# liron88/HM-16.2

Measured on AMD Instinct MI355X. Metric: CTUs/sec (enc) at 4K main10; bit-exact CU partition vs HM, higher is better.
Workload: dtype int32+f64

## Files before the change

### hm-16.2_amd/csrc/hm355_core.h

```cpp
#pragma once
#include <stddef.h>
#include "hm355_types.h"

#ifdef HM355_HOSTSIM
#include <string.h>
#include <math.h>
#include <stdlib.h>
#define HM_DEV static
#define HM_FINL static inline
#define HM_FINL_M inline
#define HM_LAMBDA_INL
#define HM_NOINLINE __attribute__((noinline))
#define HM_CONST static const
#define HM_ASSUME_LDS(p) ((void)0)
#define HM_ASSUME_GLB(p) ((void)0)
#define HM_NT 1
static inline int hm_lane() { return 0; }
#define HM_SYNC() ((void)0)
static inline uint32_t hm_wave_sum(uint32_t v) { return v; }
static inline int hm_wave_sum_i(int v) { return v; }
static inline int hm_wave_max_i(int v) { return v; }
#define HM_UNI(x) (x)
#define HM_UCALL(x) (x)
#define hm_uni_ptr(p) (p)
// ... 45 lines not shown
}
__device__ __forceinline__ uint32_t hm_wave_sum(uint32_t v) { return (uint32_t)hm_wave_sum_i((int)v); }
__device__ __forceinline__ int hm_wave_max_i(int v)
{
  int t;
  t = hm_dpp<0x111>(v, v); v = t > v ? t : v; t = hm_dpp<0x112>(v, v); v = t > v ? t : v;
  t = hm_dpp<0x114>(v, v); v = t > v ? t : v; t = hm_dpp<0x118>(v, v); v = t > v ? t : v;
  const int a = __builtin_amdgcn_readlane(v, 15), b = __builtin_amdgcn_readlane(v, 31), c = __builtin_amdgcn_readlane(v, 47), d = __builtin_amdgcn_readlane(v, 63);
  const int ab = a > b ? a : b, cd = c > d ? c : d;
  return ab > cd ? ab : cd;
}
#define HM_LDS_ADD(p, v) atomicAdd((p), (v))
#define HM_UNI(x) __builtin_amdgcn_readfirstlane((int)(x))
template <class T> __device__ __forceinline__ T *hm_uni_ptr(T *p)
{
  const unsigned long long v = (unsigned long long)p;
  const unsigned lo = (unsigned)__builtin_amdgcn_readfirstlane((int)(unsigned)v), hi = (unsigned)__builtin_amdgcn_readfirstlane((int)(unsigned)(v >> 32));
  return (T *)(((unsigned long long)hi << 32) | lo);
}
template <class T> __device__ __forceinline__ T hm_uni_struct(T v)
{
  static_assert(sizeof(T) % 4 == 0, "dword-sized aggregates only");
  int w[sizeof(T) / 4];
  __builtin_memcpy(w, &v, sizeof(T));
#pragma unroll
  for (unsigned i = 0; i < sizeof(T) / 4; i++) w[i] = __builtin_amdgcn_readfirstlane(w[i]);
  __builtin_memcpy(&v, w, sizeof(T));
  return v;
}
#define HM_ENTRY(e) do { (e) = hm_uni_ptr(e); HM_ASSUME_LDS(e); } while (0)
#define HM_UCALL(x) ((uint32_t)__builtin_amdgcn_readfirstlane((int)(x)))
#define HM_PAR_FOR(i, n) for (int i = hm_lane(); i < (n); i += HM_NT)
#define HM_PAR_FOR_XY(x, y, w, n) \
  for (int i_ = hm_lane(), sy_ = HM_NT / (w), sx_ = HM_NT - sy_ * (w), y = i_ / (w), x = i_ - y * (w); i_ < (n); \
       i_ += HM_NT, x += sx_, y += sy_, (x >= (w) ? (x -= (w), y++) : 0))
#define HM_WAVE_FOR(k) for (int k = hm_lane(), k##_once = 1; k##_once; k##_once = 0)
#define HM_LV(T, name) T name
#define HM_LVARG(T, name) const T name
#define HM_LVK(name, k) name
#define HM_LV_GET(name, i) __builtin_amdgcn_readlane((int)(name), (int)(i))
#define HM_LV_GETD(name, i) hm_readlane_d((name), (int)(i))
#define HM_LV_SET(name, i, v) ((name) = (hm_lane() == (int)(i)) ? (v) : (name))
#define HM_LV_SETD(name, i, v) ((name) = (hm_lane() == (int)(i)) ? (v) : (name))
#define HM_LV_GATHER(name, idx) __builtin_amdgcn_ds_bpermute((int)(idx) << 2, (int)(name))
#define HM_BALLOT(m, k, cond) ((m) = __ballot(cond))
#define HM_ORDERED_ADD16(acc, name) do { _Pragma("unroll") for (int k_ = 15; k_ >= 0; k_--) (acc) += hm_readlane_d((name), k_); } while (0)
#define HM_ORDERED_CHAIN16(acc, a, b, pre) do { _Pragma("unroll") for (int k_ = 15; k_ >= 0; k_--) { \
    (pre) = (hm_lane() == k_) ? (acc) : (pre); (acc) -= hm_readlane_d((a), k_); (acc) += hm_readlane_d((b), k_); } } while (0)
__device__ __forceinline__ double hm_readlane_d(double v, int i)
{ return __hiloint2double(__builtin_amdgcn_readlane(__double2hiint(v), i), __builtin_amdgcn_readlane(__double2loint(v), i)); }
#endif

#if defined(HM355_PROFILE) && !defined(HM355_HOSTSIM)
#define HM_PROF_N 45
#define HM_PROF_BEGIN(e, id) const unsigned long long prof_t0_##id = __builtin_readcyclecounter()
#define HM_PROF_END(e, id) do { (e)->prof[id] += __builtin_readcyclecounter() - prof_t0_##id; (e)->profCnt[id] += 1; } while (0)
#else
#define HM_PROF_BEGIN(e, id) ((void)0)
#define HM_PROF_END(e, id) ((void)0)
#endif
enum { PR_RDOQ = 0, PR_BITS, PR_ADI, PR_PRED, PR_FWD, PR_INV, PR_SATD35, PR_TUBLK, PR_SAVE, PR_CHROMA, PR_LUMA, PR_ENCCU, PR_TOTAL,
       PR_S4L = 32, PR_S4C, PR_D0, PR_D1, PR_D2, PR_D3, PR_NXN, PR_S8L, PR_S4LEAF, PR_S4CLEAF, PR_S8C, PR_S16L = 44,
       PR_ME_INT = 16, PR_ME_FRAC, PR_AMVP, PR_MRG_EST, PR_MC, PR_IRQ, PR_IRES, PR_MRG2N, PR_INTERCU, PR_INTRA_IN_P, PR_IQ_FULL, PR_IQ_FWD, PR_IQ_RDOQ, PR_IQ_BITS, PR_IQ_INV, PR_IQ_ENC };

#define HM_MAX_DOUBLE 1.7e+308
#define PLANAR_IDX 0
#define DC_IDX 1
#define HOR_IDX 10
#define VER_IDX 26
#define DM_CHROMA_IDX 36
#define SIZE_2Nx2N 0
#define SIZE_NxN 3
#define SIZE_NONE 8
#define MODE_INTRA 1
#define MODE_NONE 2
#define SCAN_DIAG 0
#define SCAN_HOR 1
#define SCAN_VER 2

HM_CONST uint8_t HM_NEXT_LPS[128] __attribute__((aligned(4))) = {
  1, 0, 0, 1, 2, 3, 4, 5, 4, 5, 8, 9, 8, 9, 10, 11, 12, 13, 14, 15, 16, 17, 18, 19, 18, 19, 22, 23, 22, 23, 24, 25,
  26, 27, 26, 27, 30, 31, 30, 31, 32, 33, 32, 33, 36, 37, 36, 37, 38, 39, 38, 39, 42, 43, 42, 43, 44, 45, 44, 45, 46, 47, 48, 49,
  48, 49, 50, 51, 52, 53, 52, 53, 54, 55, 54, 55, 56, 57, 58, 59, 58, 59, 60, 61, 60, 61, 60, 61, 62, 63, 64, 65, 64, 65, 66, 67,
  66, 67, 66, 67, 68, 69, 68, 69, 70, 71, 70, 71, 70, 71, 72, 73, 72, 73, 72, 73, 74, 75, 74, 75, 74, 75, 76, 77, 76, 77, 126, 127 };
HM_CONST int32_t HM_ENTROPY_BITS[128] = {
  0x07b23, 0x085f9, 0x074a0, 0x08cbc, 0x06ee4, 0x09354, 0x067f4, 0x09c1b, 0x060b0, 0x0a62a, 0x05a9c, 0x0af5b, 0x0548d, 0x0b955, 0x04f56, 0x0c2a9,
  0x04a87, 0x0cbf7, 0x045d6, 0x0d5c3, 0x04144, 0x0e01b, 0x03d88, 0x0e937, 0x039e0, 0x0f2cd, 0x03663, 0x0fc9e, 0x03347, 0x10600, 0x03050, 0x10f95,
  0x02d4d, 0x11a02, 0x02ad3, 0x12333, 0x0286e, 0x12cad, 0x02604, 0x136df, 0x02425, 0x13f48, 0x021f4, 0x149c4, 0x0203e, 0x1527b, 0x01e4d, 0x15d00,
  0x01c99, 0x166de, 0x01b18, 0x17017, 0x019a5, 0x17988, 0x01841, 0x18327, 0x016df, 0x18d50, 0x015d9, 0x19547, 0x0147c, 0x1a083, 0x0138e, 0x1a8a3,
  0x01251, 0x1b418, 0x01166, 0x1bd27, 0x01068, 0x1c77b, 0x00f7f, 0x1d18e, 0x00eda, 0x1d91a, 0x00e19, 0x1e254, 0x00d4f, 0x1ec9a, 0x00c90, 0x1f6e0,
  0x00c01, 0x1fef8, 0x00b5f, 0x208b1, 0x00ab6, 0x21362, 0x00a15, 0x21e46, 0x00988, 0x2285d, 0x00934, 0x22ea8, 0x008a8, 0x239b2, 0x0081d, 0x24577,
  0x007c9, 0x24ce6, 0x00763, 0x25663, 0x00710, 0x25e8f, 0x006a0, 0x26a26, 0x00672, 0x26f23, 0x005e8, 0x27ef8, 0x005ba, 0x284b5, 0x0055e, 0x29057,
  0x0050c, 0x29bab, 0x004c1, 0x2a674, 0x004a7, 0x2aa5e, 0x0046f, 0x2b32f, 0x0041f, 0x2c0ad, 0x003e7, 0x2ca8d, 0x003ba, 0x2d323, 0x0010c, 0x3bfbb };
HM_CONST uint8_t HM_CTX_INIT_I[HM_NUM_CTX] = {
   139, 141, 157,
   184, 154, 154, 154,
   184,
   63, 139,
   153, 138, 138,
   111, 141, 154, 154, 154,   94, 138, 182, 154, 154,
   91, 171, 134, 141,
   111, 111, 125, 110, 110, 94, 124, 108, 124, 107, 125, 141, 179, 153, 125, 107, 125, 141, 179, 153, 125, 107, 125, 141, 179, 153, 125, 141,
   140, 139, 182, 182, 152, 136, 152, 136, 153, 136, 139, 111, 136, 139, 111, 111,
   110, 110, 124, 125, 140, 153, 125, 127, 140, 109, 111, 143, 127, 111, 79,  108, 123, 63, 154, 154, 154, 154, 154, 154, 154, 154, 154, 154, 154, 154,
   110, 110, 124, 125, 140, 153, 125, 127, 140, 109, 111, 143, 127, 111, 79,  108, 123, 63, 154, 154, 154, 154, 154, 154, 154, 154, 154, 154, 154, 154,
   140, 92, 137, 138, 140, 152, 138, 139, 153, 74, 149, 92, 139, 107, 122, 152,  140, 179, 166, 182, 140, 227, 122, 197,
   138, 153, 136, 167, 152, 152,
   139, 139,
   154, 154, 154,  154, 154,  154,  154, 154, 154, 154, 154,  154, 154,
   154, 154,  154,  154,  154, 154, 154
};
HM_CONST uint8_t HM_CTX_INIT_P[HM_NUM_CTX] = {
   107, 139, 126,
   154, 139, 154, 154,
   154,
// ... 1580 lines not shown
      const int c = hm_clip3(imin, imax, coef[i]);
      int v;
      if (rightShift > 0) v = (c * scale + (1 << (rightShift - 1))) >> rightShift;
      else v = (int)((unsigned)(c * scale) << (-rightShift));
      e->bufA[y * HM_TSTRIDE + x] = hm_clip3(-32768, 32767, v);
    }
    HM_SYNC();
    if (!tskip) inv_transform(e, n, comp == 0 && n == 4, bitDepth);
    const int off = tshift == 0 ? 0 : (1 << (tshift - 1));
    HM_PAR_FOR(i, n * n) {
      const int y = i >> l2, x = i & (n - 1);
      const int v = e->bufA[y * HM_TSTRIDE + x];
      resi[y * st + x] = (Pel)(tskip ? ((v + off) >> tshift) : v);
    }
  } else {
    HM_PAR_FOR(i, n * n) { const int y = i >> l2, x = i & (n - 1); coef[i] = 0; resi[y * st + x] = 0; }
  }
  HM_SYNC();
  HM_PROF_END(e, PR_INV);
  const int maxv = (1 << bitDepth) - 1, shiftSse = (bitDepth - 8) << 1;
  uint32_t sse = 0;
  HM_PAR_FOR(i, n * n) {
    const int y = i >> l2, x = i & (n - 1);
    const int r = hm_clip3(0, maxv, pred[y * st + x] + resi[y * st + x]);
    pred[y * st + x] = (Pel)r; recQt[y * st + x] = (Pel)r; recPic[y * ps + x] = (Pel)r;
    const int d = org[y * ps + x] - r; sse += (uint32_t)((d * d) >> shiftSse);
  }
  uint32_t d = hm_wave_sum(sse);
  HM_SYNC();
  if (comp) d = (uint32_t)(e->fb.chromaWeight * (double)d);
  return d;
}

HM_DEV inline void store_intra_result_qt(Shared *e, const TU *t, int comp)
{
  const int st = HM_PLANE_STRIDE(comp), po = HM_PLANE_OFF(comp), layer = 5 - t->log2;
  const int bx = comp ? t->cx : t->x, by = comp ? t->cy : t->y;
  const TCoeff *coef = e->ws->qtCoef[layer] + po + (comp ? t->cOff : (t->cuZ + t->relZ) * 16);
  const Pel *rq = e->ws->qtRec[layer] + po + by * st + bx;
  HM_PAR_FOR(i, 16) { e->ws->tsCoef[comp][i] = coef[i]; e->ws->tsRec[comp][i] = rq[(i >> 2) * st + (i & 3)]; }
  HM_SYNC();
}
HM_DEV inline void load_intra_result_qt(Shared *e, const TU *t, int comp)
{
  const int st = HM_PLANE_STRIDE(comp), po = HM_PLANE_OFF(comp), layer = 5 - t->log2, ps = e->stride[comp];
  const int bx = comp ? t->cx : t->x, by = comp ? t->cy : t->y;
  TCoeff *coef = e->ws->qtCoef[layer] + po + (comp ? t->cOff : (t->cuZ + t->relZ) * 16);
  Pel *rq = e->ws->qtRec[layer] + po + by * st + bx;
  Pel *recPic = e->fb.rec[comp] + (e->ctuY * st + by) * ps + e->ctuX * st + bx;
  HM_PAR_FOR(i, 16) { coef[i] = e->ws->tsCoef[comp][i]; const Pel v = e->ws->tsRec[comp][i]; rq[(i >> 2) * st + (i & 3)] = v; recPic[(i >> 2) * ps + (i & 3)] = v; }
  HM_SYNC();
}

HM_DEV HM_NOINLINE void simt4_luma_leaf(Shared *e, TU tv);
template <int L2> HM_DEV HM_NOINLINE void simt_luma_winner_as_single_tu(Shared *e, TU tv);
HM_DEV HM_NOINLINE void recur_intra_coding_qt(Shared *e, TU rootv, int checkFirst)
{
  HM_ENTRY(e); checkFirst = HM_UNI(checkFirst); rootv = hm_uni_struct(rootv);
  CtuMeta *m = (&e->meta);
  RqtFrame *fr = e->rqt; int sp = 0;
  uint32_t *retDist = e->rqtRetDist, *retBits = e->rqtRetBits; double *retCost = e->rqtRetCost;
  fr[0].t = rootv; fr[0].phase = 0; retDist[0] = 0; retBits[0] = 0; retCost[0] = 0.0;
  while (sp >= 0) {
    RqtFrame *f = &fr[sp]; const TU *t = &f->t;
    const int z = t->cuZ + t->relZ, fullDepth = t->cuDepth + t->trDepth, log2 = t->log2;
    if (f->phase == 0) {
      const int nxn = m->part[t->cuZ] == SIZE_NxN;
      f->checkFull = log2 <= 5;
      f->checkSplit = log2 > tr_min_size_in_cu(6 - t->cuDepth, nxn);
      if (checkFirst && f->checkFull) f->checkSplit = 0;
      f->singleCost = HM_MAX_DOUBLE; f->singleDist = 0; f->singleCbf = 0; f->bestModeId = 0; f->singleBits = 0;
      const int checkTS = (log2 == 2) && (m->part[z] == SIZE_NxN);
      if (f->checkFull) {
        if (checkTS) {
          cabac_copy(&e->ws->slot[HM_SLOT(fullDepth, CI_QT_TRAFO_ROOT)], &e->cur);
          for (int modeId = 0; modeId < 2; modeId++) {
            double costTmp;
            par_set8(m->ts[0] + z, modeId, t->parts);
            const uint32_t distTmp = HM_UCALL(intra_coding_tu_block(e, *t, 0, modeId == 0 ? 1 : 2));
            const uint32_t cbfTmp = (m->cbf[0][z] >> t->trDepth) & 1;
            if (modeId == 1 && cbfTmp == 0) costTmp = HM_MAX_DOUBLE;
            else { const uint32_t bits = HM_UCALL(intra_bits_qt(e, *t, 1, 0)); costTmp = calc_rd_cost(e, bits, distTmp); }
            if (costTmp < f->singleCost) {
              f->singleCost = costTmp; f->singleDist = distTmp; f->singleCbf = cbfTmp; f->bestModeId = (int8_t)modeId;
              if (modeId == 0) { store_intra_result_qt(e, t, 0); cabac_copy(&e->ws->slot[HM_SLOT(fullDepth, CI_TEMP_BEST)], &e->cur); }
            }
            if (modeId == 0) cabac_copy(&e->cur, &e->ws->slot[HM_SLOT(fullDepth, CI_QT_TRAFO_ROOT)]);
          }
          par_set8(m->ts[0] + z, f->bestModeId, t->parts);
          if (f->bestModeId == 0) {
            load_intra_result_qt(e, t, 0);
            par_set8(m->cbf[0] + z, (int)(f->singleCbf << t->trDepth), t->parts);
            cabac_copy(&e->cur, &e->ws->slot[HM_SLOT(fullDepth, CI_TEMP_BEST)]);
          }
        } else if (log2 == 2 && e->P->fewWaves) {
          par_set8(m->ts[0] + z, 0, t->parts);
          HM_PROF_BEGIN(e, PR_S4LEAF);
          simt4_luma_leaf(e, *t);
          HM_PROF_END(e, PR_S4LEAF);
          f->singleDist = e->outDistY; f->singleBits = e->outBits;
          f->singleCost = calc_rd_cost(e, e->outBits, f->singleDist);
        } else if (sp == 0 && e->s8Reuse == 1) {
          e->s8Reuse = 0;
          cabac_copy(&e->ws->slot[HM_SLOT(fullDepth, CI_QT_TRAFO_ROOT)], &e->cur);
          par_set8(m->ts[0] + z, 0, t->parts);
          par_set8(m->tr + z, t->trDepth, t->parts);
          if (log2 == 3) simt_luma_winner_as_single_tu<3>(e, *t); else simt_luma_winner_as_single_tu<4>(e, *t);
          f->singleDist = e->outDistY; f->singleCbf = e->outDist;
          par_set8(m->cbf[0] + z, (int)(f->singleCbf << t->trDepth), t->parts);
          f->singleCost = calc_rd_cost(e, e->outBits, f->singleDist);
        } else if (sp == 0 && e->s8Reuse == 2) {
          e->s8Reuse = 0;
          cabac_copy(&e->ws->slot[HM_SLOT(fullDepth, CI_QT_TRAFO_ROOT)], &e->cur);
          par_set8(m->ts[0] + z, 0, t->parts);
          par_set8(m->tr + z, t->trDepth, t->parts);
          {
            const int n = 1 << log2, layer = 5 - log2;
            par_copy32(e->ws->qtCoef[layer] + z * 16, e->cc + z * 16, n * n);
            par_copy_blk(e->ws->qtRec[layer] + t->y * 64 + t->x, 64, e->ws->reco + t->y * 64 + t->x, 64, n);
          }
          f->singleCbf = e->ws->tmpCbf[0][0] & 1;
          par_set8(m->cbf[0] + z, (int)(f->singleCbf << t->trDepth), t->parts);
          f->singleDist = e->outDistY; f->singleCost = e->outRdCost;
          cabac_copy(&e->cur, &e->ws->slot[HM_SLOT(fullDepth, CI_QT_TRAFO_TEST)]);
        } else {
          if (f->checkSplit) cabac_copy(&e->ws->slot[HM_SLOT(fullDepth, CI_QT_TRAFO_ROOT)], &e->cur);
          par_set8(m->ts[0] + z, 0, t->parts);
          f->singleDist = HM_UCALL(intra_coding_tu_block(e, *t, 0, 0));
          if (f->checkSplit) f->singleCbf = (m->cbf[0][z] >> t->trDepth) & 1;
          const uint32_t bits = HM_UCALL(intra_bits_qt(e, *t, 1, 0));
          f->singleCost = calc_rd_cost(e, bits, f->singleDist); f->singleBits = bits;
        }
      }
      if (!f->checkSplit) { retDist[sp] += f->singleDist; retBits[sp] += f->singleBits; retCost[sp] += f->singleCost; sp--; continue; }
      if (f->checkFull) { cabac_copy(&e->ws->slot[HM_SLOT(fullDepth, CI_QT_TRAFO_TEST)], &e->cur); cabac_copy(&e->cur, &e->ws->slot[HM_SLOT(fullDepth, CI_QT_TRAFO_ROOT)]); }
      else cabac_copy(&e->ws->slot[HM_SLOT(fullDepth, CI_QT_TRAFO_ROOT)], &e->cur);
      f->splitCost = 0.0; f->splitDist = 0; f->splitCbf = 0; f->child = 0; f->phase = 1;
      retDist[sp + 1] = 0; retBits[sp + 1] = 0; retCost[sp + 1] = 0.0;
    }
    if (f->phase == 1) {
      int splitLost = 0;
      if (f->child > 0) {
        const TU ch = tu_child(t, f->child - 1, 0);
        f->splitCbf |= (m->cbf[0][ch.cuZ + ch.relZ] >> ch.trDepth) & 1;
        const uint32_t lbBits = retBits[sp + 1] > (uint32_t)f->child ? retBits[sp + 1] - (uint32_t)f->child : 0;
        if (f->checkFull) splitLost = !(calc_rd_cost(e, lbBits, retDist[sp + 1]) < f->singleCost);
        else if (sp == 0 && !(calc_rd_cost(e, lbBits, retDist[1]) < e->outCost)) {
          e->outDistY = 0; e->outRdCost = HM_MAX_DOUBLE; return;
        }
      }
      if (!splitLost) {
        if (f->child < 4) {
          fr[sp + 1].t = tu_child(t, f->child, 0); fr[sp + 1].phase = 0; f->child++;
          sp++; continue;
        }
        f->splitDist = retDist[sp + 1];
        if (f->splitCbf) { HM_PAR_FOR(o, t->parts) m->cbf[0][z + o] |= (uint8_t)(1 << t->trDepth); HM_SYNC(); }
        cabac_copy(&e->cur, &e->ws->slot[HM_SLOT(fullDepth, CI_QT_TRAFO_ROOT)]);
        const uint32_t splitBits = HM_UCALL(intra_bits_qt(e, *t, 1, 0));
        f->splitCost = calc_rd_cost(e, splitBits, f->splitDist);
        if (f->splitCost < f->singleCost) { retDist[sp] += f->splitDist; retBits[sp] += splitBits; retCost[sp] += f->splitCost; sp--; continue; }
      }
      cabac_copy(&e->cur, &e->ws->slot[HM_SLOT(fullDepth, CI_QT_TRAFO_TEST)]);
      par_set8(m->tr + z, t->trDepth, t->parts);
      par_set8(m->cbf[0] + z, (int)(f->singleCbf << t->trDepth), t->parts);
      par_set8(m->ts[0] + z, f->bestModeId, t->parts);
      {
        const int n = 1 << log2, layer = 5 - log2, ps = e->stride[0];
        par_copy_blk(e->fb.rec[0] + (e->ctuY * 64 + t->y) * ps + e->ctuX * 64 + t->x, ps, e->ws->qtRec[layer] + t->y * 64 + t->x, 64, n);
      }
      retDist[sp] += f->singleDist; retBits[sp] += f->singleBits; retCost[sp] += f->singleCost; sp--; continue;
    }
  }
  e->outDistY = retDist[0]; e->outRdCost = retCost[0];
}

HM_DEV inline void set_intra_result_qt(Shared *e, const TU *root)
{
  const CtuMeta *m = (&e->meta);
  for (int rel = root->relZ; rel < root->relZ + root->parts;) {
    const int z = root->cuZ + rel, trd = m->tr[z];
    const int log2 = 6 - root->cuDepth - trd, n = 1 << log2, layer = 5 - log2;
    const int parts = root->cuParts >> (2 * trd) > 0 ? root->cuParts >> (2 * trd) : 1;
    const int r = hm_z2r(z), x = (r & 15) * 4, y = (r >> 4) * 4;
    par_copy32(e->cc + z * 16, e->ws->qtCoef[layer] + z * 16, n * n);
    par_copy_blk(e->ws->reco + y * 64 + x, 64, e->ws->qtRec[layer] + y * 64 + x, 64, n);
    rel += parts;
  }
}

#include "hm355_simt.h"
#include "hm355_simt4.h"
#include "hm355_simt8.h"
#include "hm355_simt16.h"

HM_DEV HM_NOINLINE uint32_t est_intra_pred_qt(Shared *e, int cuZ, int cuDepth)
{
  HM_ENTRY(e); cuZ = HM_UNI(cuZ); cuDepth = HM_UNI(cuDepth);
  CtuMeta *m = (&e->meta); WorkSpace *ws = e->ws;
  const int cuParts = 256 >> (2 * cuDepth);
  const int nxn = m->part[cuZ] == SIZE_NxN;
  const int numPU = nxn ? 4 : 1, puParts = cuParts / numPU;
  const int puLog2 = 6 - cuDepth - nxn, n = 1 << puLog2;
  const int bitDepth = e->bitDepth, ps = e->stride[0];
  uint32_t overallDistY = 0;
  const TU root = tu_root(e, cuZ, cuDepth);
  for (int pu = 0; pu < numPU; pu++) {
    const TU t = nxn ? tu_child(&root, pu, 0) : root;
    const int z = cuZ + t.relZ;
    int numModesForFullRD = HM_INTRA_MODE_NUM_FAST[puLog2 - 1];
    int32_t *rdModeList = e->rdModeList;
    {
      const int r = hm_z2r(z);
      init_adi_pattern(e, 0, e->ctuX * 64 + t.x, e->ctuY * 64 + t.y, n, e->ctuX * 16 + (r & 15), e->ctuY * 16 + (r >> 4), n / 4, 1);
      const Pel *org = e->fb.org[0] + (e->ctuY * 64 + t.y) * ps + e->ctuX * 64 + t.x;
      Pel *pred = ws->pred + t.y * 64 + t.x;
      int preds[HM_NUM_MPM];
      const int numMpm = intra_dir_predictor(e, z, preds);
      e->mpmZ = z; e->mpmNum = numMpm; e->mpmPreds[0] = preds[0]; e->mpmPreds[1] = preds[1]; e->mpmPreds[2] = preds[2];
      const uint64_t frac0 = e->ws->slot[HM_SLOT(cuDepth, CI_CURR_BEST)].frac & 32767;
      const uint8_t st0 = e->ws->slot[HM_SLOT(cuDepth, CI_CURR_BEST)].s[C_INTRA_LUMA];
      HM_PROF_BEGIN(e, PR_SATD35);
      if (n <= 16) satd_all_modes_small(e, org, ps, n);
      else {
        for (int mode = 0; mode < 35; mode++) {
          pred_intra(e, 0, mode, n, use_filtered_refs(0, mode, n), pred, 64);
          const uint32_t sad = dist_hads(org, ps, pred, 64, n, bitDepth);
          if (hm_lane() == 0) e->satd[mode] = sad;
        }
        HM_SYNC();
      }
      {
        HM_LV(double, vCost);
        HM_WAVE_FOR(k) {
          double cost = HM_MAX_DOUBLE;
          if (k < 35) {
            int predIdx = -1;
            for (int i = 0; i < 3; i++) if (k == preds[i]) predIdx = i;
            uint64_t fb = frac0 + (uint64_t)HM_LT()->ebits[st0 ^ (predIdx != -1)];
            fb += (uint64_t)32768 * (uint64_t)(predIdx == -1 ? 5 : (predIdx ? 2 : 1));
            const uint32_t modeBits = (uint32_t)(fb >> 15);
            cost = (double)e->satd[k] + (double)modeBits * e->fb.sqrtLambda;
          }
          HM_LVK(vCost, k) = cost;
        }
        HM_WAVE_FOR(k) {
          const double ck = HM_LVK(vCost, k);
          int rank = 0;
          for (int j = 0; j < 35; j++) { const double cj = HM_LV_GETD(vCost, j); rank += (cj < ck || (cj == ck && j < k)) ? 1 : 0; }
          if (k < 35 && rank < numModesForFullRD) rdModeList[rank] = k;
        }
        HM_SYNC();
      }
      HM_PROF_END(e, PR_SATD35);
      for (int j = 0; j < numMpm; j++) {
        int included = 0;
        for (int i = 0; i < numModesForFullRD; i++) included |= (preds[j] == rdModeList[i]);
        if (!included) rdModeList[numModesForFullRD++] = preds[j];
      }
    }
    if (n == 4) {
      cabac_copy(&e->cur, &e->ws->slot[HM_SLOT(cuDepth, CI_CURR_BEST)]);
      { HM_PROF_BEGIN(e, PR_S4L); simt4_luma_pu(e, t, numModesForFullRD); HM_PROF_END(e, PR_S4L); }
      overallDistY += e->outDistY;
      if (pu != numPU - 1)
        par_copy_blk(e->fb.rec[0] + (e->ctuY * 64 + t.y) * ps + e->ctuX * 64 + t.x, ps, ws->reco + t.y * 64 + t.x, 64, n);
      continue;
    }
    int bestPUMode = 0; uint32_t bestPUDistY = 0; double bestPUCost = HM_MAX_DOUBLE;
    int firstPass = 0;
    if (n == 8 || n == 16) {
      cabac_copy(&e->cur, &e->ws->slot[HM_SLOT(cuDepth, CI_CURR_BEST)]);
      if (n == 8) { HM_PROF_BEGIN(e, PR_S8L); bestPUMode = HM_UCALL(simt_luma_first_pass<3>(e, t, numModesForFullRD)); HM_PROF_END(e, PR_S8L); }
      else { HM_PROF_BEGIN(e, PR_S16L); bestPUMode = HM_UCALL(simt_luma_first_pass<4>(e, t, numModesForFullRD)); HM_PROF_END(e, PR_S16L); }
      firstPass = numModesForFullRD;
      e->s8Reuse = 1;
    }
    for (int pass = firstPass; pass <= numModesForFullRD; pass++) {
      const int last = (pass == numModesForFullRD);
      const int orgMode = last ? bestPUMode : rdModeList[pass];
      par_set8(m->dirL + z, orgMode, puParts);
      cabac_copy(&e->cur, &e->ws->slot[HM_SLOT(cuDepth, CI_CURR_BEST)]);
      e->outCost = bestPUCost;
// ... 385 lines not shown
  if (firstBad < 0 && got.frac == e->cur.frac) return;
  g_cub_bad++;
  const CtuMeta *m = (&e->meta);
  static const char *const chromaPath[3] = { "wave-uniform", "simt4_chroma_cu", "simt8_chroma_cu16" };
  const char *closing = m->tr[cuZ] ? "split root" : (cuDepth >= 2 ? "winner's lane (s8Reuse 1)" : "parked first pass (s8Reuse 2)");
  fprintf(stderr, "CU_BITS mismatch: frame CTU %d cuZ %d depth %d class %d, luma closing: %s, chroma: %s; frac %llu, recount %llu; first context that differs %d\n",
          e->ctuAddr, cuZ, cuDepth, how, closing, chromaPath[g_cub_chroma_path], (unsigned long long)got.frac, (unsigned long long)e->cur.frac, firstBad);
}
#endif

HM_DEV HM_NOINLINE void check_rd_cost_intra(Shared *e, int cuZ, int cuDepth, int partSize)
{
  HM_ENTRY(e); cuZ = HM_UNI(cuZ); cuDepth = HM_UNI(cuDepth); partSize = HM_UNI(partSize);
  CtuMeta *m = (&e->meta); const int parts = 256 >> (2 * cuDepth);
#if defined(HM355_PROFILE) && !defined(HM355_HOSTSIM)
  const unsigned long long profCu0 = __builtin_readcyclecounter();
#endif
  init_est_data(e, cuZ, cuDepth);
  HM_PAR_FOR(i, parts) { m->part[cuZ + i] = (uint8_t)partSize; m->pred[cuZ + i] = MODE_INTRA; }
  HM_SYNC();
  HM_PROF_BEGIN(e, PR_LUMA);
  uint32_t d = HM_UCALL(est_intra_pred_qt(e, cuZ, cuDepth));
  HM_PROF_END(e, PR_LUMA);
  {
    const int r = hm_z2r(cuZ), x = (r & 15) * 4, y = (r >> 4) * 4, n = 64 >> cuDepth, ps = e->stride[0];
    par_copy_blk(e->fb.rec[0] + (e->ctuY * 64 + y) * ps + e->ctuX * 64 + x, ps, e->ws->reco + y * 64 + x, 64, n);
  }
  { HM_PROF_BEGIN(e, PR_CHROMA); d += HM_UCALL(est_intra_pred_chroma_qt(e, cuZ, cuDepth)); HM_PROF_END(e, PR_CHROMA); }
  HM_PROF_BEGIN(e, PR_ENCCU);
  const int how = cu_bits_class(e, cuZ, cuDepth, partSize);
  if (how == CUB_RECOUNT) { reset_bits(&e->cur); encode_cu_syntax(e, &e->cur, cuZ, cuDepth); }
  else cu_bits_from_passes(e, cuZ, cuDepth, how);
  HM_PROF_END(e, PR_ENCCU);
#if defined(HM355_CHECK_CU_BITS)
  cu_bits_check(e, cuZ, cuDepth, partSize, how);
#endif
  cabac_copy(&e->ws->slot[HM_SLOT(cuDepth, CI_TEMP_BEST)], &e->cur);
  e->outBits = num_bits(&e->cur); e->outDist = d;
  e->outCost = calc_rd_cost(e, e->outBits, e->outDist);
  check_dqp(e, cuZ, cuDepth);
#if defined(HM355_PROFILE) && !defined(HM355_HOSTSIM)
  { const int pid = partSize == SIZE_NxN ? PR_NXN : PR_D0 + cuDepth; e->prof[pid] += __builtin_readcyclecounter() - profCu0; e->profCnt[pid] += 1; }
#endif
}


#include "hm355_inter_cu.h"

template <class M> HM_FINL void cu_walk(Shared *e)
{
  CtuMeta *m = (&e->meta);
  CuFrame *fr = e->cuf; int sp = 0;
  fr[0].cuZ = 0; fr[0].phase = 0; fr[0].parentPart = SIZE_NONE;
  double retCost = 0; uint32_t retBits = 0, retDist = 0;
  M mode;
  while (sp >= 0) {
    CuFrame *f = &fr[sp]; const int cuDepth = sp, cuZ = f->cuZ;
    const int size = 64 >> cuDepth, parts = 256 >> (2 * cuDepth), q = parts >> 2;
    if (f->phase == 0) {
      const int r = hm_z2r(cuZ);
      const int lx = e->ctuX * 64 + (r & 15) * 4, ty = e->ctuY * 64 + (r >> 4) * 4;
      f->boundary = !((lx + size - 1 < e->width) && (ty + size - 1 < e->height));
      f->bestCost = HM_MAX_DOUBLE; f->bestBits = 0; f->bestDist = 0;
      if (mode.unsplit(e, f, cuZ, cuDepth)) { retCost = f->bestCost; retBits = f->bestBits; retDist = f->bestDist; sp--; continue; }
      init_est_data(e, cuZ, cuDepth);
      f->splitBits = 0; f->splitDist = 0; f->sub = 0; f->phase = 1;
    }
    if (f->phase == 1) {
      if (f->sub < 4) {
        const int s = f->sub++;
        const int subZ = cuZ + s * q, r = hm_z2r(subZ);
        const int sx = e->ctuX * 64 + (r & 15) * 4, sy = e->ctuY * 64 + (r >> 4) * 4;
        HM_PAR_FOR(i, q) { m->depth[subZ + i] = (uint8_t)(cuDepth + 1); m->part[subZ + i] = SIZE_NONE; m->pred[subZ + i] = MODE_NONE; }
        HM_SYNC();
        if (sx < e->width && sy < e->height) {
          if (s == 0) cabac_copy(&e->ws->slot[HM_SLOT(cuDepth + 1, CI_CURR_BEST)], &e->ws->slot[HM_SLOT(cuDepth, CI_CURR_BEST)]);
          else cabac_copy(&e->ws->slot[HM_SLOT(cuDepth + 1, CI_CURR_BEST)], &e->ws->slot[HM_SLOT(cuDepth + 1, CI_NEXT_BEST)]);
          fr[sp + 1].cuZ = (int16_t)subZ; fr[sp + 1].phase = 0;
          fr[sp + 1].parentPart = (int8_t)mode.parent_part(e, f, cuZ, cuDepth);
          f->phase = 2; sp++; continue;
        }
        continue;
      }
      if (mode.collect(e, f, cuZ, cuDepth)) { init_est_data(e, cuZ, cuDepth); f->splitBits = 0; f->splitDist = 0; f->sub = 0; continue; }
      if (!f->boundary) {
        reset_bits(&e->cur);
        enc_bin(e, &e->cur, C_SPLIT + ctx_split_flag(e, cuZ, cuDepth), m->depth[cuZ] > cuDepth);
        f->splitBits += num_bits(&e->cur);
      }
      f->splitCost = calc_rd_cost(e, f->splitBits, f->splitDist);
      if (M::kSplitPaysDqp && e->fb.dqp && cuDepth == 0 && first_coded_cu(e) < 256) {
        reset_bits(&e->cur);
        code_delta_qp(e, &e->cur, HM_UNI(e->ws->dq.ctuQp) - HM_UNI(e->ws->dq.refQp));
        f->splitBits += num_bits(&e->cur);
        f->splitCost = calc_rd_cost(e, f->splitBits, f->splitDist);
      }
      cabac_copy(&e->ws->slot[HM_SLOT(cuDepth, CI_TEMP_BEST)], &e->ws->slot[HM_SLOT(cuDepth + 1, CI_NEXT_BEST)]);
      if (f->splitCost < f->bestCost) {
        f->bestCost = f->splitCost; f->bestBits = f->splitBits; f->bestDist = f->splitDist;
        cabac_copy(&e->ws->slot[HM_SLOT(cuDepth, CI_NEXT_BEST)], &e->ws->slot[HM_SLOT(cuDepth, CI_TEMP_BEST)]);
      } else mode.take_unsplit(e, cuZ, cuDepth);
      retCost = f->bestCost; retBits = f->bestBits; retDist = f->bestDist; sp--; continue;
    }
    if (f->phase == 2) {
      f->splitBits += retBits; f->splitDist += retDist; f->phase = 1;
      if (f->sub < 4 && !f->boundary && mode.may_stop_early(e, f, cuDepth)) {
        bool laterSibling = sp == 0;
        if (sp > 0) {
          const int pq = parts, pz = fr[sp - 1].cuZ;
          for (int s2 = fr[sp - 1].sub; s2 < 4; s2++) {
            const int r2 = hm_z2r(pz + s2 * pq);
            laterSibling |= (e->ctuX * 64 + (r2 & 15) * 4 < e->width) && (e->ctuY * 64 + (r2 >> 4) * 4 < e->height);
          }
        }
        if (laterSibling && !(calc_rd_cost(e, f->splitBits, f->splitDist) < f->bestCost)) {
          mode.take_unsplit(e, cuZ, cuDepth);
          retCost = f->bestCost; retBits = f->bestBits; retDist = f->bestDist; sp--;
        }
      }
      continue;
    }
  }
  e->outCost = retCost; e->outBits = retBits; e->outDist = retDist;
}

struct WalkSolo {
  static constexpr bool kSplitPaysDqp = true;
  HM_FINL_M int unsplit(Shared *e, CuFrame *f, int cuZ, int cuDepth)
  {
    if (!f->boundary) {
      if (e->im) { HM_PROF_BEGIN(e, PR_INTERCU); compress_cu_inter_modes(e, cuZ, cuDepth, cuDepth); HM_PROF_END(e, PR_INTERCU); }
      else {
        check_rd_cost_intra(e, cuZ, cuDepth, SIZE_2Nx2N);
        double c = e->outCost; uint32_t b = e->outBits, d = e->outDist;
        if (c < f->bestCost) { f->bestCost = c; f->bestBits = b; f->bestDist = d; save_best(e, cuZ, cuDepth); cabac_copy(&e->ws->slot[HM_SLOT(cuDepth, CI_NEXT_BEST)], &e->ws->slot[HM_SLOT(cuDepth, CI_TEMP_BEST)]); }
        if (cuDepth == 3) {
          check_rd_cost_intra(e, cuZ, cuDepth, SIZE_NxN);
          c = e->outCost; b = e->outBits; d = e->outDist;
          if (c < f->bestCost) { f->bestCost = c; f->bestBits = b; f->bestDist = d; save_best(e, cuZ, cuDepth); cabac_copy(&e->ws->slot[HM_SLOT(cuDepth, CI_NEXT_BEST)], &e->ws->slot[HM_SLOT(cuDepth, CI_TEMP_BEST)]); }
        }
      }
      reset_bits(&e->cur);
      if (cuDepth != 3) enc_bin(e, &e->cur, C_SPLIT + ctx_split_flag(e, cuZ, cuDepth), 0);
      f->bestBits += num_bits(&e->cur);
      f->bestCost = calc_rd_cost(e, f->bestBits, f->bestDist);
    }
    const int noSplit = cuDepth == 3 || (e->im && !f->boundary && HM_UNI(e->P->ecu) && HM_UNI(e->ws->best[cuDepth].im.skip[cuZ]));
    if (noSplit) restore_best(e, cuZ, cuDepth);
    return noSplit;
  }
  HM_FINL_M int parent_part(Shared *e, const CuFrame *f, int cuZ, int cuDepth)
  { return (e->im && !f->boundary && e->ws->best[cuDepth].m.pred[cuZ] == MODE_INTER) ? e->ws->best[cuDepth].m.part[cuZ] : SIZE_NONE; }
  HM_FINL_M int collect(Shared *, CuFrame *, int, int) { return 0; }
  HM_FINL_M void take_unsplit(Shared *e, int cuZ, int cuDepth) { restore_best(e, cuZ, cuDepth); }
  HM_FINL_M int may_stop_early(Shared *e, CuFrame *, int) { return !e->im; }
};
HM_DEV HM_NOINLINE void compress_ctu(Shared *e) { HM_ENTRY(e); cu_walk<WalkSolo>(e); }

template <class C> HM_DEV HM_NOINLINE void encode_ctu(Shared *e, C *c, int lastCtuOfSlice)
{
  HM_ENTRY(e); lastCtuOfSlice = HM_UNI(lastCtuOfSlice); c = hm_uni_ptr(c); HM_ASSUME_LDS(c);
  const CtuMeta *m = (&e->meta);
  int16_t stackZ[4]; int8_t stackNext[4]; int sp = 0;
  stackZ[0] = 0; stackNext[0] = -1;
  while (sp >= 0) {
    const int depth = sp, z = stackZ[sp], size = 64 >> depth;
    const int r = hm_z2r(z);
    const int lx = e->ctuX * 64 + (r & 15) * 4, ty = e->ctuY * 64 + (r >> 4) * 4;
    const int inside = (lx + size - 1 < e->width) && (ty + size - 1 < e->height);
    if (stackNext[sp] < 0) {
      if (inside && depth != 3) enc_bin(e, c, C_SPLIT + ctx_split_flag(e, z, depth), m->depth[z] > depth);
      if (!((depth < m->depth[z] && depth < 3) || !inside)) {
        if (m->pred[z] == MODE_INTER) encode_cu_syntax_inter(e, c, z, depth, 1); else encode_cu_syntax(e, c, z, depth);
        const int lastX = ((lx + size) % 64 == 0) || (lx + size == e->width), lastY = ((ty + size) % 64 == 0) || (ty + size == e->height);
        if (lastX && lastY && !lastCtuOfSlice) enc_trm(e, c, 0);
        sp--; continue;
// ... 111 lines not shown
```

### hm-16.2_amd/csrc/hm355_types.h

```cpp
#pragma once
#include <stdint.h>

typedef int16_t Pel;
typedef int32_t TCoeff;

enum {
  C_SPLIT = 0, C_PART = 3, C_INTRA_LUMA = 7, C_CHROMA_PRED = 8, C_SUBDIV = 10, C_QT_CBF = 13, C_SIG_CG = 23,
  C_SIG = 27, C_LASTX = 71, C_LASTY = 101, C_ONE = 131, C_ABS = 155, C_TSKIP = 161,
   C_SKIP = 163, C_MRG_FLAG = 166, C_MRG_IDX = 167, C_PRED_MODE = 168, C_INTER_DIR = 169, C_MVD = 174, C_REF = 176,
  C_ROOT_CBF = 178, C_MVP_IDX = 179,  C_DQP = 180, HM_NUM_CTX = 183
};
struct Cabac {
  uint8_t s[184];
  uint64_t frac;
};
#define HM_CHROMA_CTX_TABLE(X) \
  X(C_CHROMA_PRED, C_SUBDIV)          \
  X(C_QT_CBF + 5, C_SIG_CG)           \
  X(C_SIG_CG + 2, C_SIG)              \
  X(C_SIG + 28, C_LASTX)              \
  X(C_LASTX + 15, C_LASTY)            \
  X(C_LASTY + 15, C_ONE)              \
  X(C_ONE + 16, C_ABS)                \
  X(C_ABS + 4, C_TSKIP)               \
// ... 17 lines not shown
  int32_t poc, isLongTerm;
  const uint8_t *predMode;
  const MvD *mv[2]; const int8_t *refIdx[2];
  int32_t refPoc[2][16], refLT[2][16];
};
struct InterPic {
  int32_t sliceType, poc, numRefIdx[2];
  RefPicDev ref[2][16];
  int32_t colFromL0, colRefIdx, tmvp, mvdL1Zero, maxMergeCand, checkLDC, cabacInitType;
  uint32_t lambdaMotionSAD, lambdaMotionSSE;
  MvD integerMv2Nx2N[2][16];
  int32_t list1ToList0[16];
};

#define HM_PLANE_OFF(c) ((c) == 0 ? 0 : ((c) == 1 ? 4096 : 5120))
#define HM_PLANE_STRIDE(c) ((c) == 0 ? 64 : 32)
#define HM_TEAM 9
#define HM_TEAM_I 5
#define HM_COEF_CTU 6144

struct Best {
  CtuMeta m;
  InterMeta im;
  TCoeff coef[HM_COEF_CTU];
  Pel reco[HM_COEF_CTU];
};

struct WorkSpace {
  Best best[4];
  Pel pred[HM_COEF_CTU], resi[HM_COEF_CTU], reco[HM_COEF_CTU];
  Pel qtRec[4][HM_COEF_CTU];
  TCoeff qtCoef[4][HM_COEF_CTU];
  MvD intMv[2][16];
  Pel tsPred[3][16], tsRec[3][16]; TCoeff tsCoef[3][16];
  double costCoeff[1024];
  Cabac slot[4 * CI_NUM + 3 + 2];
  Pel tmpPred[HM_COEF_CTU];
  Pel resiBest[HM_COEF_CTU];
  Pel mcTmp[72 * 64];
  Pel mcBlk[64 * 64];
  Pel yuvPred[2][HM_COEF_CTU];
  Pel orgBi[64 * 64];
  struct PuSearch {
    MvD mvTemp[2][16], mvPred[2][16], mvPredBi[2][16], cand[2][16][2];
    int8_t mvpIdx[2][16], mvpIdxBi[2][16], mvpNum[2][16];
    uint32_t costTempL0[16], bitsTempL0[16];
  } ps;
  struct { MvD mv[5][2]; int32_t ref[5][2]; uint8_t dir[5]; int32_t num; } mrg2N;
  uint8_t tmpTr[256], tmpCbf[3][256], tmpTs[3][256], saveCbf[3][256], saveTs[3][256];
  struct { int32_t ctuQp, refQp, flag, pad; } dq;
  TCoeff teamCoef[HM_COEF_CTU];
  InterMeta teamIm;
  MvD teamTok[3][2][16];
};

struct QpTab { int32_t qpPer[2], qpRem[2]; double errScale[2][4]; int64_t rdFactor[2]; };
struct CtuDqp {
  int8_t qp, refQp, lastQp;
  uint8_t flagOut;
  int16_t firstZ, pad;
};
struct CtuRc {
  double lambda, sqrtLambda, lambdaC;
  int64_t rdFactor[2];
  uint32_t lambdaMotionSAD, lambdaMotionSSE;
};
struct CtuRcOut { int32_t bits, qp; };
struct DqpPic {
  int32_t flagIn, sliceQp;
  const int8_t *ctuQp;
  CtuDqp *out;
  const uint8_t *rowFlag;
  QpTab tab[64];
  const CtuRc *rc;
  CtuRcOut *rcOut;
  int32_t firstCtu, pad;
};

struct Tables {
  uint8_t z2r[256], r2z[256];
  uint16_t scan[3][4][1024];
  uint16_t scanCG[3][4][64];
};

struct FrameBuf {
  Pel *org[3], *rec[3];
  CtuMeta *meta;
  TCoeff *coef;
  CtuStat *stat;
  Cabac *endState;
  uint32_t *done;
  InterMeta *imeta;
  InterPic *ip;
  MvD *intMv;
  DqpPic *dqp;
  double lambda, sqrtLambda, lambdaC, chromaWeight;
  double errScale[2][4];
  int64_t rdFactor[2];
  int32_t qp, qpPer[2], qpRem[2];
  uint32_t lambdaMotionSAD;
};

struct Params {
  int32_t width, height, bitDepth, wpp;
  int32_t wCtu, hCtu, stride[3];
  const Tables *tab;
// ... 13 lines not shown
```

Baseline: 26600.

## Reuse 32x32 TU results across 64x64 intra RQT passes

Records the distortion, bits, cbf and CABAC state of each 32x32 full-TU evaluation during the checkFirst pass of a 64x64 intra RQT. On the later non-checkFirst pass it reuses those recorded results instead of re-running intra_coding_tu_block and bit estimation. State is tracked through e->s8Reuse flags, with a two-set toggle to keep the winning mode's data. The CU walk's return values now go into e->outCost so the RQT can read them. This adds workspace storage and CABAC copies, and depends on subtle state invariants to stay bit-exact. A profiling counter for large-block SATD is also added.

```diff
diff --git a/hm-16.2_amd/csrc/hm355_core.h b/hm-16.2_amd/csrc/hm355_core.h
--- a/hm-16.2_amd/csrc/hm355_core.h
+++ b/hm-16.2_amd/csrc/hm355_core.h
@@ -121,7 +121,7 @@
 #endif
 
 #if defined(HM355_PROFILE) && !defined(HM355_HOSTSIM)
-#define HM_PROF_N 45
+#define HM_PROF_N 46
 #define HM_PROF_BEGIN(e, id) const unsigned long long prof_t0_##id = __builtin_readcyclecounter()
 #define HM_PROF_END(e, id) do { (e)->prof[id] += __builtin_readcyclecounter() - prof_t0_##id; (e)->profCnt[id] += 1; } while (0)
 #else
@@ -129,7 +129,7 @@
 #define HM_PROF_END(e, id) ((void)0)
 #endif
 enum { PR_RDOQ = 0, PR_BITS, PR_ADI, PR_PRED, PR_FWD, PR_INV, PR_SATD35, PR_TUBLK, PR_SAVE, PR_CHROMA, PR_LUMA, PR_ENCCU, PR_TOTAL,
-       PR_S4L = 32, PR_S4C, PR_D0, PR_D1, PR_D2, PR_D3, PR_NXN, PR_S8L, PR_S4LEAF, PR_S4CLEAF, PR_S8C, PR_S16L = 44,
+       PR_S4L = 32, PR_S4C, PR_D0, PR_D1, PR_D2, PR_D3, PR_NXN, PR_S8L, PR_S4LEAF, PR_S4CLEAF, PR_S8C, PR_S16L = 44, PR_SATDL ,
        PR_ME_INT = 16, PR_ME_FRAC, PR_AMVP, PR_MRG_EST, PR_MC, PR_IRQ, PR_IRES, PR_MRG2N, PR_INTERCU, PR_INTRA_IN_P, PR_IQ_FULL, PR_IQ_FWD, PR_IQ_RDOQ, PR_IQ_BITS, PR_IQ_INV, PR_IQ_ENC };
 
 #define HM_MAX_DOUBLE 1.7e+308
@@ -1816,8 +1816,40 @@
   HM_SYNC();
 }
 
+#ifdef HM355_HOSTSIM
+#include <stdio.h>
+struct Pu64ClosingStats {
+  unsigned long n[2];
+  ~Pu64ClosingStats() { if (getenv("HM355_PU64_STATS")) fprintf(stderr, "pu64 closing reused %lu evaluated %lu\n", n[0], n[1]); }
+};
+static Pu64ClosingStats g_pu64_stats;
+#define HM_PU64_STAT(i) ((void)g_pu64_stats.n[i]++)
+#else
+#define HM_PU64_STAT(i) ((void)0)
+#endif
+
 HM_DEV HM_NOINLINE void simt4_luma_leaf(Shared *e, TU tv);
 template <int L2> HM_DEV HM_NOINLINE void simt_luma_winner_as_single_tu(Shared *e, TU tv);
+HM_DEV HM_NOINLINE void pu64_record_tu(Shared *e, int k, uint32_t dist, uint32_t bits, int cbf)
+{
+  HM_ENTRY(e); k = HM_UNI(k); dist = HM_UNI(dist); bits = HM_UNI(bits); cbf = HM_UNI(cbf);
+  const int set = e->s8Reuse & 1;
+  if (hm_lane() == 0) { e->ws->pu64[set][k].dist = dist; e->ws->pu64[set][k].bits = bits; e->ws->pu64[set][k].cbf = (uint32_t)cbf; }
+  cabac_copy(&e->ws->pu64Cabac[set][k], &e->cur);
+}
+HM_DEV HM_NOINLINE void pu64_take_tu(Shared *e, TU tv, int k)
+{
+  HM_ENTRY(e); k = HM_UNI(k); tv = hm_uni_struct(tv);
+  const TU *t = &tv; CtuMeta *m = (&e->meta);
+  const int z = t->cuZ + t->relZ, set = e->s8Reuse & 1;
+  par_set8(m->ts[0] + z, 0, t->parts);
+  par_set8(m->tr + z, t->trDepth, t->parts);
+  par_copy32(e->ws->qtCoef[0] + z * 16, e->cc + z * 16, 32 * 32);
+  par_copy_blk(e->ws->qtRec[0] + t->y * 64 + t->x, 64, e->ws->reco + t->y * 64 + t->x, 64, 32);
+  e->outDistY = HM_UNI(e->ws->pu64[set][k].dist); e->outBits = HM_UNI(e->ws->pu64[set][k].bits); e->outDist = HM_UNI(e->ws->pu64[set][k].cbf);
+  par_set8(m->cbf[0] + z, (int)(e->outDist << t->trDepth), t->parts);
+  cabac_copy(&e->cur, &e->ws->pu64Cabac[set][k]);
+}
 HM_DEV HM_NOINLINE void recur_intra_coding_qt(Shared *e, TU rootv, int checkFirst)
 {
   HM_ENTRY(e); checkFirst = HM_UNI(checkFirst); rootv = hm_uni_struct(rootv);
@@ -1825,6 +1857,10 @@
   RqtFrame *fr = e->rqt; int sp = 0;
   uint32_t *retDist = e->rqtRetDist, *retBits = e->rqtRetBits; double *retCost = e->rqtRetCost;
   fr[0].t = rootv; fr[0].phase = 0; retDist[0] = 0; retBits[0] = 0; retCost[0] = 0.0;
+  if (rootv.log2 == 6) {
+    if (checkFirst) { if (!(e->outCost < HM_MAX_DOUBLE)) e->s8Reuse = 4; }
+    else e->s8Reuse = e->s8Reuse >= 4 ? 6 | ((e->s8Reuse & 1) ^ 1) : 0;
+  }
   while (sp >= 0) {
     RqtFrame *f = &fr[sp]; const TU *t = &f->t;
     const int z = t->cuZ + t->relZ, fullDepth = t->cuDepth + t->trDepth, log2 = t->log2;
@@ -1887,6 +1923,12 @@
           par_set8(m->cbf[0] + z, (int)(f->singleCbf << t->trDepth), t->parts);
           f->singleDist = e->outDistY; f->singleCost = e->outRdCost;
           cabac_copy(&e->cur, &e->ws->slot[HM_SLOT(fullDepth, CI_QT_TRAFO_TEST)]);
+        } else if (sp == 1 && e->s8Reuse >= 6) {
+          HM_PU64_STAT(0);
+          if (f->checkSplit) cabac_copy(&e->ws->slot[HM_SLOT(fullDepth, CI_QT_TRAFO_ROOT)], &e->cur);
+          pu64_take_tu(e, *t, fr[0].child - 1);
+          f->singleDist = e->outDistY; f->singleBits = e->outBits; f->singleCbf = e->outDist;
+          f->singleCost = calc_rd_cost(e, f->singleBits, f->singleDist);
         } else {
           if (f->checkSplit) cabac_copy(&e->ws->slot[HM_SLOT(fullDepth, CI_QT_TRAFO_ROOT)], &e->cur);
           par_set8(m->ts[0] + z, 0, t->parts);
@@ -1894,6 +1936,10 @@
           if (f->checkSplit) f->singleCbf = (m->cbf[0][z] >> t->trDepth) & 1;
           const uint32_t bits = HM_UCALL(intra_bits_qt(e, *t, 1, 0));
           f->singleCost = calc_rd_cost(e, bits, f->singleDist); f->singleBits = bits;
+          if (sp == 1 && log2 == 5) {
+            if (e->s8Reuse >= 4) pu64_record_tu(e, fr[0].child - 1, f->singleDist, bits, (m->cbf[0][z] >> t->trDepth) & 1);
+            else if (!checkFirst) HM_PU64_STAT(1);
+          }
         }
       }
       if (!f->checkSplit) { retDist[sp] += f->singleDist; retBits[sp] += f->singleBits; retCost[sp] += f->singleCost; sp--; continue; }
@@ -1910,6 +1956,7 @@
         const uint32_t lbBits = retBits[sp + 1] > (uint32_t)f->child ? retBits[sp + 1] - (uint32_t)f->child : 0;
         if (f->checkFull) splitLost = !(calc_rd_cost(e, lbBits, retDist[sp + 1]) < f->singleCost);
         else if (sp == 0 && !(calc_rd_cost(e, lbBits, retDist[1]) < e->outCost)) {
+          if (e->s8Reuse >= 6) e->s8Reuse = 0;
           e->outDistY = 0; e->outRdCost = HM_MAX_DOUBLE; return;
         }
       }
@@ -1923,7 +1970,10 @@
         cabac_copy(&e->cur, &e->ws->slot[HM_SLOT(fullDepth, CI_QT_TRAFO_ROOT)]);
         const uint32_t splitBits = HM_UCALL(intra_bits_qt(e, *t, 1, 0));
         f->splitCost = calc_rd_cost(e, splitBits, f->splitDist);
-        if (f->splitCost < f->singleCost) { retDist[sp] += f->splitDist; retBits[sp] += splitBits; retCost[sp] += f->splitCost; sp--; continue; }
+        if (f->splitCost < f->singleCost) {
+          if (sp == 1 && e->s8Reuse >= 6) e->s8Reuse = 0;
+          retDist[sp] += f->splitDist; retBits[sp] += splitBits; retCost[sp] += f->splitCost; sp--; continue;
+        }
       }
       cabac_copy(&e->cur, &e->ws->slot[HM_SLOT(fullDepth, CI_QT_TRAFO_TEST)]);
       par_set8(m->tr + z, t->trDepth, t->parts);
@@ -1936,6 +1986,7 @@
       retDist[sp] += f->singleDist; retBits[sp] += f->singleBits; retCost[sp] += f->singleCost; sp--; continue;
     }
   }
+  if (rootv.log2 == 6) { if (!checkFirst) e->s8Reuse = 0; else if (retCost[0] < e->outCost) e->s8Reuse ^= 1; }
   e->outDistY = retDist[0]; e->outRdCost = retCost[0];
 }
 
@@ -1987,12 +2038,14 @@
       HM_PROF_BEGIN(e, PR_SATD35);
       if (n <= 16) satd_all_modes_small(e, org, ps, n);
       else {
+        HM_PROF_BEGIN(e, PR_SATDL);
         for (int mode = 0; mode < 35; mode++) {
           pred_intra(e, 0, mode, n, use_filtered_refs(0, mode, n), pred, 64);
           const uint32_t sad = dist_hads(org, ps, pred, 64, n, bitDepth);
           if (hm_lane() == 0) e->satd[mode] = sad;
         }
         HM_SYNC();
+        HM_PROF_END(e, PR_SATDL);
       }
       {
         HM_LV(double, vCost);
@@ -2484,8 +2537,8 @@
   CtuMeta *m = (&e->meta);
   CuFrame *fr = e->cuf; int sp = 0;
   fr[0].cuZ = 0; fr[0].phase = 0; fr[0].parentPart = SIZE_NONE;
-  double retCost = 0; uint32_t retBits = 0, retDist = 0;
   M mode;
+  e->outCost = 0; e->outBits = 0; e->outDist = 0;
   while (sp >= 0) {
     CuFrame *f = &fr[sp]; const int cuDepth = sp, cuZ = f->cuZ;
     const int size = 64 >> cuDepth, parts = 256 >> (2 * cuDepth), q = parts >> 2;
@@ -2494,7 +2547,7 @@
       const int lx = e->ctuX * 64 + (r & 15) * 4, ty = e->ctuY * 64 + (r >> 4) * 4;
       f->boundary = !((lx + size - 1 < e->width) && (ty + size - 1 < e->height));
       f->bestCost = HM_MAX_DOUBLE; f->bestBits = 0; f->bestDist = 0;
-      if (mode.unsplit(e, f, cuZ, cuDepth)) { retCost = f->bestCost; retBits = f->bestBits; retDist = f->bestDist; sp--; continue; }
+      if (mode.unsplit(e, f, cuZ, cuDepth)) { e->outCost = f->bestCost; e->outBits = f->bestBits; e->outDist = f->bestDist; sp--; continue; }
       init_est_data(e, cuZ, cuDepth);
       f->splitBits = 0; f->splitDist = 0; f->sub = 0; f->phase = 1;
     }
@@ -2532,10 +2585,10 @@
         f->bestCost = f->splitCost; f->bestBits = f->splitBits; f->bestDist = f->splitDist;
         cabac_copy(&e->ws->slot[HM_SLOT(cuDepth, CI_NEXT_BEST)], &e->ws->slot[HM_SLOT(cuDepth, CI_TEMP_BEST)]);
       } else mode.take_unsplit(e, cuZ, cuDepth);
-      retCost = f->bestCost; retBits = f->bestBits; retDist = f->bestDist; sp--; continue;
+      e->outCost = f->bestCost; e->outBits = f->bestBits; e->outDist = f->bestDist; sp--; continue;
     }
     if (f->phase == 2) {
-      f->splitBits += retBits; f->splitDist += retDist; f->phase = 1;
+      f->splitBits += e->outBits; f->splitDist += e->outDist; f->phase = 1;
       if (f->sub < 4 && !f->boundary && mode.may_stop_early(e, f, cuDepth)) {
         bool laterSibling = sp == 0;
         if (sp > 0) {
@@ -2547,13 +2600,12 @@
         }
         if (laterSibling && !(calc_rd_cost(e, f->splitBits, f->splitDist) < f->bestCost)) {
           mode.take_unsplit(e, cuZ, cuDepth);
-          retCost = f->bestCost; retBits = f->bestBits; retDist = f->bestDist; sp--;
+          e->outCost = f->bestCost; e->outBits = f->bestBits; e->outDist = f->bestDist; sp--;
         }
       }
       continue;
     }
   }
-  e->outCost = retCost; e->outBits = retBits; e->outDist = retDist;
 }
 
 struct WalkSolo {
diff --git a/hm-16.2_amd/csrc/hm355_types.h b/hm-16.2_amd/csrc/hm355_types.h
--- a/hm-16.2_amd/csrc/hm355_types.h
+++ b/hm-16.2_amd/csrc/hm355_types.h
@@ -93,6 +93,8 @@
   TCoeff teamCoef[HM_COEF_CTU];
   InterMeta teamIm;
   MvD teamTok[3][2][16];
+  struct { uint32_t dist, bits, cbf, pad; } pu64[2][4];
+  Cabac pu64Cabac[2][4];
 };
 
 struct QpTab { int32_t qpPer[2], qpRem[2]; double errScale[2][4]; int64_t rdFactor[2]; };
```

Result: faster. 26880, median of 6 (+1.0%).
